# BarnitaSharma/Part-based-3D-Reconstruction

Measured on AMD Instinct MI355X. Metric: Mvoxel/s carved (semantic carve, 1024^3 grid), higher is better.
Workload: dtype u8

## Files before the change

### include/pb3d.h

```cpp
#ifndef PB3D_H
#define PB3D_H

#include <stddef.h>
#include <stdint.h>

#ifdef __cplusplus
extern "C" {
#endif

typedef struct pb3d_ctx pb3d_ctx;
typedef struct pb3d_event pb3d_event;

enum {
    PB3D_OK = 0,
    PB3D_EINVAL = -1,
    PB3D_ENODEVICE = -2,
    PB3D_ENOMEM = -3,
    PB3D_EUNSUPPORTED = -4,
    PB3D_ECOMM = -5,
    PB3D_EINDEX = -6
};

int pb3d_version(void);
const char* pb3d_last_error(void);
// ... 14 lines not shown
int pb3d_d2d(pb3d_ctx* ctx, void* dst, const void* src, size_t bytes);
int pb3d_event_create(pb3d_ctx* ctx, pb3d_event** ev);
int pb3d_event_record(pb3d_ctx* ctx, pb3d_event* ev);
int pb3d_event_elapsed_ms(pb3d_ctx* ctx, pb3d_event* start, pb3d_event* stop, float* ms);
void pb3d_event_destroy(pb3d_event* ev);

int pb3d_rotinv(int angle_deg, double M[9]);
int pb3d_offset(const double M[9], const int64_t shape[3], double off[3]);

int pb3d_carve_mask_dev(pb3d_ctx* ctx, const uint8_t* d_grid, int64_t W, int64_t H, int64_t D, int C,
                        const uint8_t* d_mask_wh, uint8_t* d_out);
int pb3d_carve_mask(pb3d_ctx* ctx, const uint8_t* grid, int64_t W, int64_t H, int64_t D, int C,
                    const uint8_t* mask_wh, uint8_t* out);

int pb3d_rotate_carve_dev(pb3d_ctx* ctx, const uint8_t* d_occ, int64_t W, int64_t H, int64_t D,
                          const double M[9], const double off[3], const uint8_t* d_mask_wh, uint8_t* d_out);
int pb3d_rotate_carve(pb3d_ctx* ctx, const uint8_t* occ, int64_t W, int64_t H, int64_t D,
                      const double M[9], const double off[3], const uint8_t* mask_wh, uint8_t* out);

int pb3d_process_grid_dev(pb3d_ctx* ctx, const uint8_t* d_occ, int64_t W, int64_t H, int64_t D,
                          const uint8_t* d_mask_wh, int angle_interval, uint8_t* d_out, uint8_t* d_tmp);
int pb3d_process_grid(pb3d_ctx* ctx, const uint8_t* occ, int64_t W, int64_t H, int64_t D,
                      const uint8_t* mask_wh, int angle_interval, uint8_t* out);

enum {
    PB3D_I8 = 1, PB3D_U8 = 2, PB3D_I16 = 3, PB3D_U16 = 4, PB3D_I32 = 5, PB3D_U32 = 6, PB3D_I64 = 7, PB3D_U64 = 8,
    PB3D_F32 = 9, PB3D_F64 = 10, PB3D_C64 = 11, PB3D_C128 = 12
};
size_t pb3d_dtype_bytes(int dtype);
int pb3d_process_grid_typed_dev(pb3d_ctx* ctx, const void* d_grid, int dtype, int64_t W, int64_t H, int64_t D, const uint8_t* d_mask_wh,
                                int angle_interval, void* d_out, void* d_tmp);

int pb3d_occupancy_dev(pb3d_ctx* ctx, const uint8_t* d_grid_rgb, int64_t nvox, uint8_t* d_occ);
int pb3d_occupancy(pb3d_ctx* ctx, const uint8_t* grid_rgb, int64_t nvox, uint8_t* occ);

int pb3d_color_apply_dev(pb3d_ctx* ctx, const uint8_t* d_carved, int64_t W, int64_t H, int64_t D,
                         const uint8_t* d_rgb_hw3, uint8_t* d_out);
int pb3d_color_apply(pb3d_ctx* ctx, const uint8_t* carved, int64_t W, int64_t H, int64_t D,
                     const uint8_t* rgb_hw3, uint8_t* out);

int pb3d_global_carve_dev(pb3d_ctx* ctx, const uint8_t* d_bin_hw, const uint8_t* d_rgb_hw3, int64_t h, int64_t w,
                          int angle_interval, int64_t x0, int64_t x1, uint8_t* d_out_slab);
int pb3d_global_carve(pb3d_ctx* ctx, const uint8_t* bin_hw, const uint8_t* rgb_hw3, int64_t h, int64_t w,
                      int angle_interval, uint8_t* out);

int pb3d_part_carve_dev(pb3d_ctx* ctx, const uint8_t* d_colored, int64_t W, int64_t H, int64_t D,
// ... 372 lines not shown
```

### part-based-3d-reconstruction_amd/csrc/ctx.hip

```cpp
#include <cmath>
#include <cstdlib>

#include <string>

#include "pb3d_internal.h"

static int pool_flush(pb3d_ctx* ctx);

static thread_local char g_err[512] = "";

void pb3d_set_error(const char* fmt, ...) {
    va_list ap;
    va_start(ap, fmt);
    vsnprintf(g_err, sizeof(g_err), fmt, ap);
    va_end(ap);
}

extern "C" {

int pb3d_version(void) { return 101; }

int64_t pb3d_sync_count(pb3d_ctx* ctx) { return ctx ? (int64_t)ctx->sync_count : -1; }

const char* pb3d_last_error(void) { return g_err; }
// ... 84 lines not shown
                (void)hipEventDestroy(ctx->s32_ev);
                (void)hipStreamDestroy(ctx->stream);
                free(ctx);
                return PB3D_EINVAL;
            }
        }
    }
    *out = ctx;
    return PB3D_OK;
}

namespace {
struct Knob { const char* name; int pb3d_ctx::*field; int lo, hi; const char* what; };
const Knob kKnobs[] = {
    {"sliced", &pb3d_ctx::tune_sliced, 0, 1, "0 (rotation steps on 0/1 data run bit-sliced) or 1 (never: byte chain)"},
    {"rot90_wide", &pb3d_ctx::tune_rot90_wide, 0, 2, "0 (choose), 1 or 2 (the 128-tile / 128-byte-segment kernels)"},
    {"rot90_fill", &pb3d_ctx::tune_rot90_fill, 0, 64, "a count of workgroups per CU (0 = the built-in rule)"},
    {"rot90_order", &pb3d_ctx::tune_rot90_order, 0, 1, "0 (a plane chunk per XCD) or 1 (plain x-fastest order)"},
    {"rot90_flat", &pb3d_ctx::tune_rot90_flat, 0, 2, "0 (choose), 1 (row-wise tile kernel) or 2 (flat on whole-line streams only)"},
    {"rot90_mask_block", &pb3d_ctx::tune_rot90_mask_block, 0, 1, "0 (mask bytes once into LDS) or 1 (per plane / segment)"},
    {"s32_gpw", &pb3d_ctx::tune_s32_gpw, 0, 1 << 20, "a count of plane groups"},
    {"s32_order", &pb3d_ctx::tune_s32_order, 0, 1, "0 (plane groups fastest) or 1 (x fastest)"},
    {"s32_fuse_last", &pb3d_ctx::tune_s32_fuse_last, 0, 1, "0 (fused) or 1 (table step)"},
    {"ccl_blocks", &pb3d_ctx::tune_ccl_blocks, 0, 1 << 20, "a count of workgroups per CU"},
    {"ccl_init_blocks", &pb3d_ctx::tune_ccl_init_blocks, 0, 1 << 20, "a count of workgroups per CU"},
    {"ccl_tilecols", &pb3d_ctx::tune_ccl_tilecols, 0, 64, "at most 64"},
    {"ccl_merge", &pb3d_ctx::tune_ccl_merge, 0, 1, "0 (tile kernels) or 1 (pairwise kernel)"},
    {"cluster_cell", &pb3d_ctx::tune_cluster_cell, 0, 2, "0 (the built-in rule), 1 (two points per cell) or 2 (cell edge above eps)"},
    {"cluster_timing", &pb3d_ctx::tune_cluster_timing, 0, 1, "0 or 1 (time the passes of a clustering with events)"},
    {"voxelize_timing", &pb3d_ctx::tune_voxelize_timing, 0, 1, "0 or 1 (time the two passes of a voxelization with events)"},
    {"render_timing", &pb3d_ctx::tune_render_timing, 0, 1, "0 or 1 (time the passes of a mesh rendering with events)"},
    {"iso_timing", &pb3d_ctx::tune_iso_timing, 0, 1, "0 or 1 (time the passes of an isosurface count and fill with events)"},
    {"simplify_timing", &pb3d_ctx::tune_simplify_timing, 0, 1, "0 or 1 (time the passes of a mesh simplification with events)"},
    {"inside_timing", &pb3d_ctx::tune_inside_timing, 0, 1, "0 or 1 (time the index build and the query of a containment test with events)"},
    {"inside_order", &pb3d_ctx::tune_inside_order, 0, 1, "0 (queries in input order) or 1 (in the cell order of the index)"},
    {"inside_table", &pb3d_ctx::tune_inside_table, 0, 1, "0 (set-ups recomputed from the corner table) or 1 (read from a table of finished set-ups)"},
    {"raycast_timing", &pb3d_ctx::tune_raycast_timing, 0, 1, "0 or 1 (time the index build and the query of a ray cast with events)"},
    {"raycast_stats", &pb3d_ctx::tune_raycast_stats, 0, 1, "0 or 1 (count hits, bad rays, face tests and cells of a ray cast for pb3d_cast_rays_last)"},
    {"orient_tile",&pb3d_ctx::tune_orient_tile, 0, 1, "0 (128-pixel tiles where they apply) or 1 (never)"},
    {"global_composed", &pb3d_ctx::tune_global_composed, 0, 1, "0 (mask bits -> sliced chain -> colours) or 1 (ones -> process -> colour)"},
    {"per_job", &pb3d_ctx::tune_per_job, 0, 1, "0 (merged / fused forms) or 1 (job by job)"},
    {"no_table_cache", &pb3d_ctx::tune_no_table_cache, 0, 1, "0 (tables cached across calls) or 1 (rebuilt every call)"},
    {"part90_inflight", &pb3d_ctx::tune_part90_inflight, 0, 44, "10 UA + UE with UA, UE in 1, 2, 4 (0 = the default 2 / 4)"},
    {"crop_ablate", &pb3d_ctx::tune_crop_ablate, 0, 1 << 20, "ablation switches of k_crop_chain"},
    {"uncap", &pb3d_ctx::tune_uncap, 0, 1, "0 or 1 (every grid-stride kernel as one workgroup per tile)"},
};
// ... 285 lines not shown
```

### part-based-3d-reconstruction_amd/csrc/pb3d_internal.h

```cpp
#pragma once
#include <hip/hip_runtime.h>

#include <cstdarg>
#include <cstdint>
#include <cstdio>
#include <cstring>
#include <initializer_list>
#include <type_traits>

#include "pb3d.h"

typedef uint8_t u8;
typedef int64_t i64;
typedef uint64_t u64;
typedef uint32_t u32;

enum pb3d_slot : int {
    PB3D_SLOT_HOST_IN0 = 0,
    PB3D_SLOT_HOST_OUT0 = 1,
    PB3D_SLOT_HOST_IN1 = 2,
    PB3D_SLOT_HOST_OUT1 = PB3D_SLOT_HOST_IN1,
    PB3D_SLOT_HOST_IN2 = 3,
    PB3D_SLOT_HOST_OUT2 = PB3D_SLOT_HOST_IN2,
    PB3D_SLOT_HOST_TMP = PB3D_SLOT_HOST_IN2,
// ... 241 lines not shown
    int device;
    int cus;
    hipStream_t stream;
    bool orient_lds_set;
    bool guided_lds_set;
    int tune_rot90_fill;
    int tune_rot90_order;
    int tune_rot90_flat;
    int tune_rot90_mask_block;
    int tune_orient_tile;
    int tune_global_composed;
    int tune_per_job;
    int tune_no_table_cache;
    int tune_part90_inflight;
    int tune_crop_ablate;
    int tune_uncap;
    int tune_sliced;
    int tune_rot90_wide;
    bool rot90w_lds_set;
    bool part90_lds_set;
    bool rot90wf_lds_set;
    int tune_s32_order;
    int tune_s32_fuse_last;
    int tune_s32_gpw;
    int tune_ccl_blocks;
    int tune_ccl_init_blocks;
    int tune_ccl_tilecols;
    int tune_ccl_merge;
    int tune_cluster_cell;
    int tune_cluster_timing;
    struct ClusterLast { bool valid, timed; float ms[5]; i64 cells[3]; } cluster_last;
    int tune_voxelize_timing;
    struct VoxelizeLast { bool valid, timed; float ms[2]; } voxelize_last;
    int tune_render_timing;
    struct RenderLast { bool valid, timed; float ms[5]; i64 stats[4]; } render_last;
    int tune_iso_timing;
    struct IsoLast { bool count_timed, fill_timed; float ms[4]; } iso_last;
    int tune_simplify_timing;
    struct SimplifyLast { bool valid, timed; float ms[5]; i64 counts[3]; } simplify_last;
    int tune_inside_timing;
    int tune_inside_order;
    int tune_inside_table;
    struct InsideLast { bool valid, timed; float ms[2]; i64 info[4]; } inside_last;
    int tune_raycast_timing;
    int tune_raycast_stats;
    struct RaycastLast { bool counted, timed; float ms[2]; i64 stats[6]; } raycast_last;
    void* scratch[PB3D_SLOT_COUNT];
    size_t scratch_bytes[PB3D_SLOT_COUNT];
    void* pinned;
    size_t pinned_bytes;
    void* stage;
    size_t stage_bytes, stage_head;
    u64 sync_count;
    struct PointsArgs { const void* grid; i64 A0, A1, A2, n, C, ncolors, stride; u8 colors[3 * 32]; };
    struct { pb3d_pair pair; PointsArgs a; } pts_dev, pts;
    struct MeshArgs { const void* grid; i64 A0, A1, A2, nv, nf, C, stride; };
    struct { pb3d_pair pair; MeshArgs a; } mesh_dev, mesh;
    struct IsoArgs { const void* vol; i64 n0, n1, n2, nv, nf; u64 level_bits, divisor_bits; };
    struct { pb3d_pair pair; IsoArgs a; } iso_dev, iso;
    struct { pb3d_pair pair; int ox, oy, oz; i64 X, Y, Z, n; } deform;
    struct ValidCache { void* buf; u64 gen; i64 W, D; double p[8]; } valid_cache;
    struct S32Cache { bool valid; u64 gen; i64 W, D; int ns; double p[32 * 8]; } s32_cache;
    hipEvent_t s32_ev;
    struct CclLast { bool valid; const void* labels; const void* bits; i64 rows, A2, P; u64 gen; bool members_only; int K, C; u32 colors[PB3D_CCL_MAX_COLORS]; } ccl_last;
    struct IcpIndex { bool valid; const void* tgt; i64 nt; int f64; u64 gen[3]; pb3d_nn_index ix; } icp_index;
    struct MeshGridLast { bool valid; i64 cells[3], entries, coarsenings; } mesh_grid_last;
    struct PoolBlock { void* p; size_t bytes; u64 stamp; };
    PoolBlock pool_free[PB3D_POOL_SLOTS];
    int pool_nfree;
    PoolBlock pool_live[PB3D_POOL_LIVE];
    int pool_nlive;
    size_t pool_cached, pool_cap;
    u64 pool_stamp;
    u64 scratch_gen;
    u64 scratch_slot_gen[PB3D_SLOT_COUNT];
    u64 scratch_use[PB3D_SLOT_COUNT];
    void* rccl_lib;
    void* rccl_comm;
    int rank, nranks;
};

void pb3d_set_error(const char* fmt, ...);

#define PB3D_HIP(call)                                                                          \
    do {                                                                                        \
// ... 159 lines not shown
```

### part-based-3d-reconstruction_amd/csrc/rot_common.h

```cpp
#pragma once
#include "pb3d_internal.h"

namespace {

struct RotParams {
    double m00, m01, m02, off0;
    double m20, m21, m22, off2;
};

struct Cell {
    double wx0, wx1, wz0, wz1;
    int s0, s2;
};

__device__ __forceinline__ double coord(double x, double z, double ma, double mb, double mc, double off) {
    double c = __dadd_rn(0.0, __dmul_rn(x, ma));
    c = __dadd_rn(c, __dmul_rn(0.0, mb));
    c = __dadd_rn(c, __dmul_rn(z, mc));
    return __dadd_rn(c, off);
}

__device__ __forceinline__ Cell make_cell(const RotParams& p, i64 x, i64 z, i64 W, i64 D) {
    Cell c;
    const double cc0 = coord((double)x, (double)z, p.m00, p.m01, p.m02, p.off0);
// ... 11 lines not shown
    return c;
}

__device__ __forceinline__ u32 lut_of(const Cell& c) {
    const double p00 = __dmul_rn(c.wx0, c.wz0), p01 = __dmul_rn(c.wx0, c.wz1), p10 = __dmul_rn(c.wx1, c.wz0),
                 p11 = __dmul_rn(c.wx1, c.wz1);
    u32 lut = 0;
#pragma unroll
    for (int b = 1; b < 16; ++b) {
        double acc = 0.0;
        if (b & 1) acc = __dadd_rn(acc, p00);
        if (b & 2) acc = __dadd_rn(acc, p01);
        if (b & 4) acc = __dadd_rn(acc, p10);
        if (b & 8) acc = __dadd_rn(acc, p11);
        if (acc > 0.0 && __dadd_rn(acc, 0.5) >= 1.0) lut |= 1u << b;
    }
    return lut;
}

__device__ __forceinline__ u32 bsel(u32 sel, u32 a, u32 b) { return (sel & a) | (~sel & b); }

__device__ __forceinline__ u32 sbit(u32 x, int k) { u32 r; asm("v_bfe_i32 %0, %1, %2, 1" : "=v"(r) : "v"(x), "n"(k)); return r; }
__device__ __forceinline__ u32 vbfi(u32 s, u32 a, u32 b) { u32 r; asm("v_bfi_b32 %0, %1, %2, %3" : "=v"(r) : "v"(s), "v"(a), "v"(b)); return r; }
__device__ __forceinline__ u32 lut_apply32(u32 lut, u32 t00, u32 t01, u32 t10, u32 t11) {
    u32 g[8], h[4];
    g[0] = vbfi(t00, sbit(lut, 1), sbit(lut, 0));   g[1] = vbfi(t00, sbit(lut, 3), sbit(lut, 2));
    g[2] = vbfi(t00, sbit(lut, 5), sbit(lut, 4));   g[3] = vbfi(t00, sbit(lut, 7), sbit(lut, 6));
    g[4] = vbfi(t00, sbit(lut, 9), sbit(lut, 8));   g[5] = vbfi(t00, sbit(lut, 11), sbit(lut, 10));
    g[6] = vbfi(t00, sbit(lut, 13), sbit(lut, 12)); g[7] = vbfi(t00, sbit(lut, 15), sbit(lut, 14));
#pragma unroll
    for (int j = 0; j < 4; ++j) h[j] = vbfi(t01, g[2 * j + 1], g[2 * j]);
    const u32 m0 = vbfi(t10, h[1], h[0]), m1 = vbfi(t10, h[3], h[2]);
    return vbfi(t11, m1, m0);
}

__device__ __forceinline__ u32 pperm(u32 hi, u32 lo, u32 sel) { return __builtin_amdgcn_perm(hi, lo, sel); }
__device__ __forceinline__ void tr4x4(u32 a0, u32 a1, u32 a2, u32 a3, u32 v[4]) {
    const u32 l01 = pperm(a1, a0, 0x05010400u), h01 = pperm(a1, a0, 0x07030602u);
    const u32 l23 = pperm(a3, a2, 0x05010400u), h23 = pperm(a3, a2, 0x07030602u);
    v[0] = pperm(l23, l01, 0x05040100u); v[1] = pperm(l23, l01, 0x07060302u);
    v[2] = pperm(h23, h01, 0x05040100u); v[3] = pperm(h23, h01, 0x07060302u);
}

}
```

### part-based-3d-reconstruction_amd/csrc/sliced.hip

```cpp
#include "rot_common.h"
#include "wave.h"

namespace {

typedef u32 u32x4 __attribute__((ext_vector_type(4)));
typedef u32 u32x2 __attribute__((ext_vector_type(2)));
typedef u32x2 u32x2_a1 __attribute__((aligned(1)));

constexpr int ST = 64;
constexpr int STHREADS = 256;
constexpr int SROWS = 96;
#ifndef PB3D_SPITCH
#define PB3D_SPITCH 101
#endif
constexpr int SPITCH = PB3D_SPITCH;
constexpr int SMAXU = 9;
constexpr int SMAXSTEPS = 32;

struct STile {
    int bx0, bz0, nrows, nunits, fits, pad0, pad1, pad2;
    u32 ugoff[SMAXU * STHREADS];
    unsigned short uloff[SMAXU * STHREADS];
    u32 cellw[16 * STHREADS];
};
static_assert(sizeof(STile) % 16 == 0, "STile is read with 16-byte loads");

struct StepParams { RotParams p[SMAXSTEPS]; };

__global__ __launch_bounds__(256) void k_s32_maskbits(const u8* __restrict__ mask_wh, i64 W, i64 H, int G, u32* __restrict__ bits, int* __restrict__ flag) {
    const i64 i = (i64)blockIdx.x * 256 + threadIdx.x;
    if (i == 0 && flag) *flag = 0;
    if (i >= (i64)G * W) return;
    const i64 g = i / W, x = i - g * W, y0 = 32 * g;
    u32 b = 0;
    if (y0 + 32 <= H) {
        typedef u32 u32x4_m1 __attribute__((ext_vector_type(4), aligned(1)));
        const u32x4_m1 lo = *(const u32x4_m1*)(mask_wh + x * H + y0), hi = *(const u32x4_m1*)(mask_wh + x * H + y0 + 16);
        const u32 w[8] = {lo.x, lo.y, lo.z, lo.w, hi.x, hi.y, hi.z, hi.w};
#pragma unroll
        for (int j = 0; j < 8; ++j) {
            const u32 t = w[j];
            const u32 z = (((t & 0x7f7f7f7fu) + 0x7f7f7f7fu) | t) & 0x80808080u;
            b |= (((z >> 7) * 0x01020408u) >> 24) << (4 * j);
// ... 285 lines not shown
            const u32 R = c[0], G = c[1], B = c[2];
            const u32 C0 = R | (G << 8) | (B << 16) | (R << 24), C1 = G | (B << 8) | (R << 16) | (G << 24), C2 = B | (R << 8) | (G << 16) | (B << 24);
#pragma unroll
            for (int j = 0; j < 4; ++j) rgb4((v[j][q >> 3] >> (q & 7)) & 0x01010101u, C0, C1, C2, o + 3 * j);
        }
        if (!fullrow) {
            if (live) {
                u8* dp = out + rowbase + (i64)q * D * 3 + 48 * zp;
                for (int bb = 0; bb < 48 && 3 * z + bb < 3 * D; ++bb) dp[bb] = (u8)(o[bb >> 2] >> (8 * (bb & 3)));
            }
            continue;
        }
#pragma unroll
        for (int k = 0; k < 3; ++k) { u32x4 t4; t4.x = o[4 * k]; t4.y = o[4 * k + 1]; t4.z = o[4 * k + 2]; t4.w = o[4 * k + 3]; win[wv][3 * lane + k] = t4; }
#pragma unroll
        for (int k = 0; k < 3; ++k) {
            const int cidx = 8 * k + zp;
            const u32x4 t4 = win[wv][grp + cidx];
            if (rowlive) *(u32x4_a1*)(out + rowbase + (i64)q * D * 3 + 16 * cidx) = t4;
        }
    }
}

__global__ __launch_bounds__(STHREADS) void k_s32_prep(StepParams sp, i64 W, i64 D, i64 Dp, int ntz, STile* __restrict__ tiles) {
    __shared__ int bb[4];
    __shared__ int rmin[SROWS], rmax[SROWS];
    __shared__ int ustart[SROWS + 1];
    __shared__ int rc0[SROWS];
    const int tid = threadIdx.x;
    const RotParams p = sp.p[blockIdx.y];
    const int t = (int)blockIdx.x;
    STile* o = tiles + (i64)blockIdx.y * gridDim.x + t;
    const i64 x0 = (i64)(t / ntz) * ST, z0 = (i64)(t % ntz) * ST;
    if (tid == 0) { bb[0] = 0x7fffffff; bb[1] = -1; bb[2] = 0x7fffffff; bb[3] = -1; }
    if (tid < SROWS) { rmin[tid] = 0x7fffffff; rmax[tid] = -1; }
    __syncthreads();
    const int tz = tid & 15, jr = tid >> 4;
    int s0[16], s2[16];
    u32 lut[16];
    int mn0 = 0x7fffffff, mx0 = -1, mn2 = 0x7fffffff, mx2 = -1;
#pragma unroll
    for (int i = 0; i < 4; ++i)
#pragma unroll
        for (int c = 0; c < 4; ++c) {
            const int k = 4 * i + c;
            const i64 x = x0 + jr + 16 * i, z = z0 + 4 * tz + c;
            s0[k] = -1; s2[k] = 0; lut[k] = 0;
            if (x < W && z < D) {
                const Cell cl = make_cell(p, x, z, W, D);
                if (cl.s0 >= 0) {
                    s0[k] = cl.s0; s2[k] = cl.s2;
                    lut[k] = lut_of(cl) | (cl.wx1 != 0.0 ? 1u << 16 : 0u) | (cl.wz1 != 0.0 ? 1u << 17 : 0u);
                    const int e0 = cl.s0 + (int)((lut[k] >> 16) & 1u), e2 = cl.s2 + (int)((lut[k] >> 17) & 1u);
                    mn0 = min(mn0, cl.s0); mx0 = max(mx0, e0); mn2 = min(mn2, cl.s2); mx2 = max(mx2, e2);
                }
            }
        }
// ... 24 lines not shown
                rc0[r] = 0;
                if (r < nrows && fits && rmax[r] >= 0) {
                    rc0[r] = (rmin[r] - bz0) >> 2;
                    n[h] = ((rmax[r] - bz0) >> 2) - ((rmin[r] - bz0) >> 2) + 1;
                }
            }
        }
        const int inc0 = wave_incl_scan(n[0]), inc1 = wave_incl_scan(n[1]);
        const int tot0 = __shfl(inc0, 63);
        ustart[tid] = inc0 - n[0];
        if (tid + 64 <= SROWS) ustart[tid + 64] = tot0 + inc1 - n[1];
    }
    __syncthreads();
    int nunits = (any_valid && fits) ? ustart[SROWS] : 0;
    if (nunits > SMAXU * STHREADS) { fits = false; nunits = 0; }
    if (fits && tid < nrows) {
        const int u0 = ustart[tid], u1 = ustart[tid + 1];
        for (int u = u0; u < u1; ++u) {
            const int cu = rc0[tid] + (u - u0);
            o->ugoff[u] = (u32)(((i64)bx0 + tid) * Dp + bz0 + 4 * cu);
            o->uloff[u] = (unsigned short)(tid * SPITCH + 4 * cu);
        }
    }
#pragma unroll
    for (int k = 0; k < 16; ++k) {
        u32 w = 0;
        if (fits && s0[k] >= 0) w = (lut[k] << 16) | (u32)((s0[k] - bx0) * SPITCH + (s2[k] - bz0));
        o->cellw[k * STHREADS + tid] = w;
    }
    if (tid == 0) { o->bx0 = bx0; o->bz0 = bz0; o->nrows = nrows; o->nunits = nunits; o->fits = fits ? 1 : 0; o->pad0 = o->pad1 = o->pad2 = 0; }
}

__global__ __launch_bounds__(STHREADS, 4) void k_s32_step(const u32* __restrict__ in, u32* __restrict__ out, const u32* __restrict__ mbits,
                                                           const STile* __restrict__ tiles, i64 W, i64 Dp, int G, int ntz, int ntiles, int gpw,
                                                           int nchunks) {
    __shared__ u32 tile[SROWS * SPITCH];
    const int tid = threadIdx.x;
    const int slot = (int)(blockIdx.x >> 3);
    const int t = slot % ntiles;
    const int chunk = (slot / ntiles) * 8 + (int)(blockIdx.x & 7u);
    if (chunk >= nchunks) return;
    const STile* ti = tiles + t;
    const i64 x0 = (i64)(t / ntz) * ST, z0 = (i64)(t % ntz) * ST;
    const int g_beg = chunk * gpw, g_end = g_beg + gpw < G ? g_beg + gpw : G;
    const int nunits = ti->nunits;
    u32 ug[SMAXU], ul[SMAXU];
#pragma unroll
    for (int j = 0; j < SMAXU; ++j) {
        const int u = tid + STHREADS * j;
        ug[j] = 0xffffffffu; ul[j] = 0;
        if (u < nunits) { ug[j] = ti->ugoff[u]; ul[j] = ti->uloff[u]; }
    }
    u32 cw[16];
#pragma unroll
    for (int i = 0; i < 16; ++i) cw[i] = ti->cellw[i * STHREADS + tid];
    const int tz = tid & 15, jr = tid >> 4;
    const i64 zc = z0 + 4 * tz;
    const bool zok = zc < Dp;
    u32x4 v[SMAXU];
    auto load_group = [&](int g) {
        const u32* src = in + (i64)g * W * Dp;
#pragma unroll
        for (int j = 0; j < SMAXU; ++j)
            if (ug[j] != 0xffffffffu) v[j] = *(const u32x4*)(src + ug[j]);
    };
    load_group(g_beg);
    for (int g = g_beg; g < g_end; ++g) {
#pragma unroll
        for (int j = 0; j < SMAXU; ++j)
            if (ug[j] != 0xffffffffu) { u32* d = tile + ul[j]; d[0] = v[j].x; d[1] = v[j].y; d[2] = v[j].z; d[3] = v[j].w; }
        __syncthreads();
        if (g + 1 < g_end) load_group(g + 1);
#pragma unroll
        for (int i = 0; i < 4; ++i) {
            u32 R[4];
#pragma unroll
            for (int c = 0; c < 4; ++c) {
                const u32 w = cw[4 * i + c];
                const u32* tp = tile + (w & 0xffffu);
                R[c] = lut_apply32(w >> 16, tp[0], tp[1], tp[SPITCH], tp[SPITCH + 1]);
            }
            const i64 x = x0 + jr + 16 * i;
            if (x < W && zok) {
                const u32 m = mbits[(i64)g * W + x];
                u32x4 r; r.x = R[0] & m; r.y = R[1] & m; r.z = R[2] & m; r.w = R[3] & m;
                *(u32x4*)(out + ((i64)g * W + x) * Dp + zc) = r;
            }
        }
        __syncthreads();
    }
}

static bool step_fits(const double M[9]) {
    const double ext0 = fabs(M[0]) + fabs(M[2]), ext2 = fabs(M[6]) + fabs(M[8]);
    return ext0 <= 1.4143 && ext2 <= 1.4143;
}

}

static int s32_chain(pb3d_ctx* ctx, const u8* d_occ, i64 W, i64 H, i64 D, const u8* d_mask_wh, int angle_interval, u8* d_out, const u8* d_rgb_hw3,
                     int known_binary, int* took, const double* Mx = nullptr, const double* offx = nullptr) {
    *took = 0;
    const int nrot = Mx ? 1 : 90 / angle_interval;
// ... 35 lines not shown
            const bool nt = W * H * D >= (i64)256 << 20;
#define PB3D_SLICE(WH, NTL) hipLaunchKernelGGL((k_s32_slice<WH, NTL>), dim3((total + 255u) / 256u), dim3(256), 0, ctx->stream, d_occ, (u32*)A, Mx ? (const u32*)nullptr : (const u32*)mb, W, H, D, Dp, mzb, mw, total, flag, mg, gfast)
            if (D % 16 == 0) { if (nt) PB3D_SLICE(true, true); else PB3D_SLICE(true, false); }
            else { if (nt) PB3D_SLICE(false, true); else PB3D_SLICE(false, false); }
#undef PB3D_SLICE
        } else {
            const u32 tq = (u32)((i64)G * W * (Dp / 4));
            hipLaunchKernelGGL(k_s32_fill, dim3((tq + 255u) / 256u), dim3(256), 0, ctx->stream, (u32*)A, (const u32*)mb, D, Dp, pb3d_make_magic((u32)(Dp / 4)), tq);
        }
        PB3D_CHECK_LAUNCH();
        int* hflag = (int*)((char*)ctx->pinned + pb3d_pinned_bytes - pb3d_pinned_flag);
        if (!known_binary) {
            PB3D_HIP(hipMemcpyAsync(hflag, flag, sizeof(int), hipMemcpyDeviceToHost, ctx->stream));
            PB3D_HIP(hipEventRecord(ctx->s32_ev, ctx->stream));
        }
        int gpw = ctx->tune_s32_gpw > 0 ? ctx->tune_s32_gpw : 1;
        if (ctx->tune_s32_gpw <= 0)
            while (gpw < G && (i64)ntiles * ((G + gpw - 1) / gpw) > (i64)ctx->cus * 16) ++gpw;
        const int nchunks = (G + gpw - 1) / gpw;
        const i64 nblk = 8ll * ntiles * ((nchunks + 7) / 8);
        PB3D_REQUIRE(nblk < (1ll << 31), "pb3d_process_grid: grid too large");
        u32 *src = (u32*)A, *dst = (u32*)B;
        bool checked = known_binary != 0;
        int nrot_tab = nrot;
        u32* vbits = nullptr;
        int vnw = 0, pc0 = 0, pc2 = 0;
        if (!Mx && nrot * angle_interval == 90 && ctx->tune_s32_fuse_last != 1 && H <= 65535ll * 32) {
            double M[9], off[3];
            PB3D_TRY(pb3d_rotinv(90, M));
            PB3D_TRY(pb3d_offset(M, shape, off));
            bool rot90 = false;
            if (pb3d_is_perm_step(M, off, W, D)) {
                PB3D_TRY(pb3d_perm_valid_table(ctx, M, off, W, D, &vbits, &vnw, &pc0, &pc2, &rot90));
                if (rot90) nrot_tab = nrot - 1; else vbits = nullptr;
            }
        }
        for (int s0 = 0; s0 < nrot_tab; s0 += SMAXSTEPS) {
            const int ns = nrot_tab - s0 < SMAXSTEPS ? nrot_tab - s0 : SMAXSTEPS;
            memset(&sp, 0, sizeof(sp));
            for (int k = 0; k < ns; ++k) {
                double M[9], off[3];
                if (Mx) { memcpy(M, Mx, sizeof(M)); memcpy(off, offx, sizeof(off)); }
                else {
                    PB3D_TRY(pb3d_rotinv((s0 + k + 1) * angle_interval, M));
                    PB3D_TRY(pb3d_offset(M, shape, off));
                }
                if (!step_fits(M)) return PB3D_EUNSUPPORTED;
                sp.p[k] = RotParams{M[0], M[1], M[2], off[0], M[6], M[7], M[8], off[2]};
            }
            void* tp;
            PB3D_TRY(pb3d_scratch(ctx, PB3D_SLOT_S32_TILE_PROGRAMS, (size_t)ns * ntiles * sizeof(STile), &tp));
            pb3d_ctx::S32Cache& sc = ctx->s32_cache;
            const bool hit = ctx->tune_no_table_cache != 1 && sc.valid && sc.gen == ctx->scratch_gen && sc.W == W && sc.D == D && sc.ns == ns &&
                             memcmp(sc.p, sp.p, sizeof(RotParams) * (size_t)ns) == 0;
            if (!hit) {
                sc.valid = false;
                hipLaunchKernelGGL(k_s32_prep, dim3((unsigned)ntiles, (unsigned)ns), dim3(STHREADS), 0, ctx->stream, sp, W, D, Dp, ntz, (STile*)tp);
                PB3D_CHECK_LAUNCH();
                static_assert(sizeof(sc.p) == sizeof(sp.p), "S32Cache holds one StepParams");
                memcpy(sc.p, sp.p, sizeof(sp.p));
                sc.W = W; sc.D = D; sc.ns = ns; sc.gen = ctx->scratch_gen; sc.valid = nrot_tab <= SMAXSTEPS;
            }
            for (int k = 0; k < ns; ++k) {
                hipLaunchKernelGGL(k_s32_step, dim3((unsigned)nblk), dim3(STHREADS), 0, ctx->stream, (const u32*)src, dst, (const u32*)mb,
                                   (const STile*)tp + (i64)k * ntiles, W, Dp, G, ntz, ntiles, gpw, nchunks);
                u32* t2 = src; src = dst; dst = t2;
            }
            PB3D_CHECK_LAUNCH();
        }
        if (vbits && d_rgb_hw3) {
            const int utz = (int)((D + UZ - 1) / UZ), utx = (int)((W + UX - 1) / UX);
            hipLaunchKernelGGL(k_s32_unslice90_rgb, dim3((unsigned)(utz * utx), (unsigned)G), dim3(256), 0, ctx->stream, (const u32*)src, d_out, d_rgb_hw3,
                               (const u32*)mb, (const u32*)vbits, vnw, W, H, D, Dp, pc0, pc2, utz);
        } else if (vbits) {
            const int utz = (int)((D + UZ - 1) / UZ), utx = (int)((W + UX - 1) / UX);
            hipLaunchKernelGGL(k_s32_unslice90, dim3((unsigned)(utz * utx), (unsigned)G), dim3(256), 0, ctx->stream, (const u32*)src, d_out, (const u32*)mb,
                               (const u32*)vbits, vnw, W, H, D, Dp, pc0, pc2, utz);
        } else if (d_rgb_hw3)
            hipLaunchKernelGGL(k_s32_unslice_rgb, dim3((total + 255u) / 256u), dim3(256), 0, ctx->stream, (const u32*)src, d_out, d_rgb_hw3, W, H, D, Dp, mzb, mw,
                               total);
        else
// ... 8 lines not shown
    };
    rc = body();
    (void)pb3d_dev_free(ctx, A);
    (void)pb3d_dev_free(ctx, B);
    if (rc == PB3D_EUNSUPPORTED) return PB3D_OK;
    if (rc == PB3D_OK) *took = 1;
    return rc;
}

int pb3d_process_grid_sliced(pb3d_ctx* ctx, const u8* d_occ, i64 W, i64 H, i64 D, const u8* d_mask_wh, int angle_interval, u8* d_out,
                             int known_binary, int* took) {
    return s32_chain(ctx, d_occ, W, H, D, d_mask_wh, angle_interval, d_out, nullptr, known_binary, took);
}

int pb3d_global_carve_sliced(pb3d_ctx* ctx, const u8* d_mask_wh, const u8* d_rgb_hw3, i64 W, i64 H, i64 D, int angle_interval, u8* d_out_rgb,
                             int* took) {
    return s32_chain(ctx, nullptr, W, H, D, d_mask_wh, angle_interval, d_out_rgb, d_rgb_hw3, 1, took);
}

int pb3d_rotate_step_sliced(pb3d_ctx* ctx, const u8* d_occ, i64 W, i64 H, i64 D, const double M[9], const double off[3], const u8* d_mask_wh, u8* d_out,
                            int* took) {
    return s32_chain(ctx, d_occ, W, H, D, d_mask_wh, 90, d_out, nullptr, 0, took, M, off);
}
```

### part-based-3d-reconstruction_amd/pb3d/_lib.py

```python
import ctypes as C
import os
import threading

import numpy as np

_HERE = os.path.dirname(os.path.abspath(__file__))
LIB_PATH = os.environ.get("PB3D_LIB_PATH") or os.path.join(_HERE, "libpb3d.so")

u8p = C.POINTER(C.c_uint8)
i64 = C.c_int64
i64p = C.POINTER(C.c_int64)
dblp = C.POINTER(C.c_double)
intp = C.POINTER(C.c_int)
vp = C.c_void_p

_SIGNATURES = {
    "pb3d_version": [],
    "pb3d_last_error": [],
    "pb3d_device_count": [intp],
    "pb3d_create": [C.c_int, C.POINTER(vp)],
    "pb3d_destroy": [vp],
    "pb3d_make_current": [vp],
    "pb3d_device_info": [vp, C.c_char_p, C.c_int, intp, i64p],
    "pb3d_sync": [vp],
    "pb3d_set_tuning": [vp, C.c_char_p, C.c_int],
    "pb3d_dev_alloc": [vp, C.c_size_t, C.POINTER(vp)],
    "pb3d_dev_free": [vp, vp],
    "pb3d_dev_memset": [vp, vp, C.c_int, C.c_size_t],
    "pb3d_h2d": [vp, vp, vp, C.c_size_t],
    "pb3d_d2h": [vp, vp, vp, C.c_size_t],
    "pb3d_h2d_async": [vp, vp, vp, C.c_size_t],
    "pb3d_sync_count": [vp],
    "pb3d_d2d": [vp, vp, vp, C.c_size_t],
    "pb3d_event_create": [vp, C.POINTER(vp)],
    "pb3d_event_record": [vp, vp],
    "pb3d_event_elapsed_ms": [vp, vp, vp, C.POINTER(C.c_float)],
    "pb3d_event_destroy": [vp],
    "pb3d_rotinv": [C.c_int, dblp],
    "pb3d_offset": [dblp, i64p, dblp],
    "pb3d_carve_mask_dev": [vp, vp, i64, i64, i64, C.c_int, vp, vp],
    "pb3d_carve_mask": [vp, u8p, i64, i64, i64, C.c_int, u8p, u8p],
    "pb3d_rotate_carve_dev": [vp, vp, i64, i64, i64, dblp, dblp, vp, vp],
    "pb3d_rotate_carve": [vp, u8p, i64, i64, i64, dblp, dblp, u8p, u8p],
    "pb3d_process_grid_dev": [vp, vp, i64, i64, i64, vp, C.c_int, vp, vp],
    "pb3d_process_grid": [vp, u8p, i64, i64, i64, u8p, C.c_int, u8p],
    "pb3d_dtype_bytes": [C.c_int],
    "pb3d_process_grid_typed_dev": [vp, vp, C.c_int, i64, i64, i64, vp, C.c_int, vp, vp],
    "pb3d_occupancy_dev": [vp, vp, i64, vp],
    "pb3d_occupancy": [vp, u8p, i64, u8p],
    "pb3d_color_apply_dev": [vp, vp, i64, i64, i64, vp, vp],
    "pb3d_color_apply": [vp, u8p, i64, i64, i64, u8p, u8p],
    "pb3d_global_carve_dev": [vp, vp, vp, i64, i64, C.c_int, i64, i64, vp],
    "pb3d_global_carve": [vp, u8p, u8p, i64, i64, C.c_int, u8p],
    "pb3d_part_carve_dev": [vp, vp, i64, i64, i64, vp, vp, intp, intp, C.c_int, vp],
    "pb3d_part_carve": [vp, u8p, i64, i64, i64, u8p, u8p, intp, intp, C.c_int, u8p],
    "pb3d_points_count_dev": [vp, vp, i64, i64, i64, C.c_int, u8p, C.c_int, C.c_int, i64p],
    "pb3d_points_fill_dev": [vp, vp, i64, i64, i64, C.c_int, u8p, C.c_int, C.c_int, i64, vp, vp],
    "pb3d_points_extract_dev": [vp, vp, i64, i64, i64, C.c_int, u8p, C.c_int, i64, vp, vp, i64p],
    "pb3d_points_count": [vp, u8p, i64, i64, i64, C.c_int, u8p, C.c_int, C.c_int, i64p],
    "pb3d_points_fill": [vp, i64, C.POINTER(C.c_float), u8p],
    "pb3d_mesh_count_dev": [vp, vp, i64, i64, i64, C.c_int, C.c_int, i64p, i64p],
    "pb3d_mesh_fill_dev": [vp, vp, i64, i64, i64, C.c_int, C.c_int, i64, i64, vp, vp, vp, vp],
    "pb3d_mesh_colors_dev": [vp, vp, i64, i64, i64, C.c_int, C.c_int, vp, i64, vp],
    "pb3d_mesh_count": [vp, u8p, i64, i64, i64, C.c_int, C.c_int, i64p, i64p],
    "pb3d_mesh_fill": [vp, i64, i64, vp, vp, vp, vp],
    "pb3d_iso_count_resident": [vp, vp, i64, i64, i64, C.c_double, C.c_float, i64p, i64p],
    "pb3d_iso_fill_resident": [vp, vp, i64, i64, i64, C.c_double, C.c_float, i64, i64, vp, vp],
    "pb3d_iso_count": [vp, vp, i64, i64, i64, C.c_double, C.c_float, i64p, i64p],
# ... 131 lines not shown
    "pb3d_render_last_ms": [vp, dblp],
    "pb3d_cast_rays_resident": [vp, vp, vp, C.c_int, i64, vp, C.c_int, i64, vp, C.c_int, i64, C.c_double, C.c_double, C.c_int, vp, vp, vp, vp],
    "pb3d_cast_rays_last": [vp, i64p],
    "pb3d_cast_rays_last_ms": [vp, dblp],
}
class IouRow(C.Structure):
    _fields_ = [("pred", vp), ("gt", vp), ("gate", vp), ("pred_bits", C.c_uint32), ("gt_bits", C.c_uint32), ("gate_bits", C.c_uint32)]


_VIEW_FIELDS = [("R", C.c_double * 9), ("cam", C.c_double * 3), ("f", C.c_double), ("cx", C.c_double), ("cy", C.c_double),
                ("prec", C.c_int * 4), ("Himg", C.c_int), ("Wimg", C.c_int)]


class CarveView(C.Structure):
    _fields_ = _VIEW_FIELDS + [("d_maskbits", vp)]


class PaintView(C.Structure):
    _fields_ = _VIEW_FIELDS + [("d_image", vp), ("d_zbuf", vp)]


PRESENCE_BYTES = 1 << 21

_RESTYPES = {"pb3d_dtype_bytes": C.c_size_t, "pb3d_sync_count": C.c_int64, "pb3d_last_error": C.c_char_p, "pb3d_destroy": None, "pb3d_event_destroy": None}

EXPORTED_SYMBOLS = tuple(_SIGNATURES)

_lib = None
_ctx = None
_lock = threading.Lock()


class Pb3dError(RuntimeError):
    pass


def load():
    global _lib
    if _lib is None:
        if not os.path.exists(LIB_PATH):
            raise ImportError(f"{LIB_PATH} is missing: build it with `python -c 'import __graft_entry__ as g; g.build()'` "
                              "(pb3d has no CPU fallback)")
        lib = C.CDLL(LIB_PATH)
        for name, args in _SIGNATURES.items():
            fn = getattr(lib, name)
            fn.argtypes = args
            fn.restype = _RESTYPES.get(name, C.c_int)
# ... 18 lines not shown


def default_device():
    for key in ("PB3D_DEVICE", "LOCAL_RANK"):
        if os.environ.get(key, "").isdigit():
            return int(os.environ[key])
    return 0


def ctx():
    global _ctx
    with _lock:
        if _ctx is None:
            h = vp()
            check(load().pb3d_create(default_device(), C.byref(h)))
            _ctx = h
    return _ctx


def set_tuning(name, value):
    check(load().pb3d_set_tuning(ctx(), name.encode(), int(value)))


def reset():
    global _ctx
    with _lock:
        if _ctx is not None:
            load().pb3d_destroy(_ctx)
            _ctx = None


def _ptr(b):
    if b is None or isinstance(b, C.c_void_p):
        return b
    return C.c_void_p(b.ptr)


def p_u8(a):
    return a.ctypes.data_as(u8p)


def p_dbl(a):
    return a.ctypes.data_as(dblp)


def as_u8(a, what):
# ... 9 lines not shown
```

Baseline: 1.142 million.

## Use canonical tile programs in bit-sliced rotation step for common 4-input tables

Classifies each cell's 16-bit lookup table in the prep kernel as one of eight canonical forms (selecting a corner or majority/threshold functions), and when all cells of a wave qualify, the step kernel evaluates them with a short bitop3/bfi sequence instead of the general 15-instruction mux tree. Cell words now store byte offsets plus a 3-bit code, with a zeroed LDS pad for empty cells. It also adds counters and API calls reporting canonical versus general waves. This adds wave-uniform branching and prep work, and only helps when the interpolation tables match the canonical set.

```diff
diff --git a/include/pb3d.h b/include/pb3d.h
--- a/include/pb3d.h
+++ b/include/pb3d.h
@@ -60,6 +60,9 @@
                           const uint8_t* d_mask_wh, int angle_interval, uint8_t* d_out, uint8_t* d_tmp);
 int pb3d_process_grid(pb3d_ctx* ctx, const uint8_t* occ, int64_t W, int64_t H, int64_t D,
                       const uint8_t* mask_wh, int angle_interval, uint8_t* out);
+int pb3d_s32_last_build(pb3d_ctx* ctx, int64_t* n_canonical_waves, int64_t* n_general_waves);
+int pb3d_s32_canon_of(uint32_t table16, uint32_t* code);
+uint32_t pb3d_s32_canon_table(uint32_t code);
 
 enum {
     PB3D_I8 = 1, PB3D_U8 = 2, PB3D_I16 = 3, PB3D_U16 = 4, PB3D_I32 = 5, PB3D_U32 = 6, PB3D_I64 = 7, PB3D_U64 = 8,
diff --git a/part-based-3d-reconstruction_amd/csrc/ctx.hip b/part-based-3d-reconstruction_amd/csrc/ctx.hip
--- a/part-based-3d-reconstruction_amd/csrc/ctx.hip
+++ b/part-based-3d-reconstruction_amd/csrc/ctx.hip
@@ -130,6 +130,7 @@
     {"s32_gpw", &pb3d_ctx::tune_s32_gpw, 0, 1 << 20, "a count of plane groups"},
     {"s32_order", &pb3d_ctx::tune_s32_order, 0, 1, "0 (plane groups fastest) or 1 (x fastest)"},
     {"s32_fuse_last", &pb3d_ctx::tune_s32_fuse_last, 0, 1, "0 (fused) or 1 (table step)"},
+    {"s32_tree", &pb3d_ctx::tune_s32_tree, 0, 1, "0 (canonical tile programs where the tables allow) or 1 (the general tree everywhere)"},
     {"ccl_blocks", &pb3d_ctx::tune_ccl_blocks, 0, 1 << 20, "a count of workgroups per CU"},
     {"ccl_init_blocks", &pb3d_ctx::tune_ccl_init_blocks, 0, 1 << 20, "a count of workgroups per CU"},
     {"ccl_tilecols", &pb3d_ctx::tune_ccl_tilecols, 0, 64, "at most 64"},
diff --git a/part-based-3d-reconstruction_amd/csrc/pb3d_internal.h b/part-based-3d-reconstruction_amd/csrc/pb3d_internal.h
--- a/part-based-3d-reconstruction_amd/csrc/pb3d_internal.h
+++ b/part-based-3d-reconstruction_amd/csrc/pb3d_internal.h
@@ -287,6 +287,7 @@
     bool rot90wf_lds_set;
     int tune_s32_order;
     int tune_s32_fuse_last;
+    int tune_s32_tree;
     int tune_s32_gpw;
     int tune_ccl_blocks;
     int tune_ccl_init_blocks;
@@ -325,7 +326,8 @@
     struct { pb3d_pair pair; IsoArgs a; } iso_dev, iso;
     struct { pb3d_pair pair; int ox, oy, oz; i64 X, Y, Z, n; } deform;
     struct ValidCache { void* buf; u64 gen; i64 W, D; double p[8]; } valid_cache;
-    struct S32Cache { bool valid; u64 gen; i64 W, D; int ns; double p[32 * 8]; } s32_cache;
+    struct S32Cache { bool valid; u64 gen; i64 W, D; int ns, tree; double p[32 * 8]; } s32_cache;
+    bool s32_built;
     hipEvent_t s32_ev;
     struct CclLast { bool valid; const void* labels; const void* bits; i64 rows, A2, P; u64 gen; bool members_only; int K, C; u32 colors[PB3D_CCL_MAX_COLORS]; } ccl_last;
     struct IcpIndex { bool valid; const void* tgt; i64 nt; int f64; u64 gen[3]; pb3d_nn_index ix; } icp_index;
diff --git a/part-based-3d-reconstruction_amd/csrc/rot_common.h b/part-based-3d-reconstruction_amd/csrc/rot_common.h
--- a/part-based-3d-reconstruction_amd/csrc/rot_common.h
+++ b/part-based-3d-reconstruction_amd/csrc/rot_common.h
@@ -57,16 +57,41 @@
 
 __device__ __forceinline__ u32 sbit(u32 x, int k) { u32 r; asm("v_bfe_i32 %0, %1, %2, 1" : "=v"(r) : "v"(x), "n"(k)); return r; }
 __device__ __forceinline__ u32 vbfi(u32 s, u32 a, u32 b) { u32 r; asm("v_bfi_b32 %0, %1, %2, %3" : "=v"(r) : "v"(s), "v"(a), "v"(b)); return r; }
+template <int B = 0>
 __device__ __forceinline__ u32 lut_apply32(u32 lut, u32 t00, u32 t01, u32 t10, u32 t11) {
     u32 g[8], h[4];
-    g[0] = vbfi(t00, sbit(lut, 1), sbit(lut, 0));   g[1] = vbfi(t00, sbit(lut, 3), sbit(lut, 2));
-    g[2] = vbfi(t00, sbit(lut, 5), sbit(lut, 4));   g[3] = vbfi(t00, sbit(lut, 7), sbit(lut, 6));
-    g[4] = vbfi(t00, sbit(lut, 9), sbit(lut, 8));   g[5] = vbfi(t00, sbit(lut, 11), sbit(lut, 10));
-    g[6] = vbfi(t00, sbit(lut, 13), sbit(lut, 12)); g[7] = vbfi(t00, sbit(lut, 15), sbit(lut, 14));
+    g[0] = vbfi(t00, sbit(lut, B + 1), sbit(lut, B + 0));   g[1] = vbfi(t00, sbit(lut, B + 3), sbit(lut, B + 2));
+    g[2] = vbfi(t00, sbit(lut, B + 5), sbit(lut, B + 4));   g[3] = vbfi(t00, sbit(lut, B + 7), sbit(lut, B + 6));
+    g[4] = vbfi(t00, sbit(lut, B + 9), sbit(lut, B + 8));   g[5] = vbfi(t00, sbit(lut, B + 11), sbit(lut, B + 10));
+    g[6] = vbfi(t00, sbit(lut, B + 13), sbit(lut, B + 12)); g[7] = vbfi(t00, sbit(lut, B + 15), sbit(lut, B + 14));
 #pragma unroll
     for (int j = 0; j < 4; ++j) h[j] = vbfi(t01, g[2 * j + 1], g[2 * j]);
     const u32 m0 = vbfi(t10, h[1], h[0]), m1 = vbfi(t10, h[3], h[2]);
     return vbfi(t11, m1, m0);
+}
+
+__host__ __device__ inline u32 canon_table(u32 code) {
+    switch (code & 7u) {
+        case 0: return 0xeaa8u; case 1: return 0xecc8u; case 2: return 0xf8e0u; case 3: return 0xfe80u;
+        case 4: return 0xaaaau; case 5: return 0xccccu; case 6: return 0xf0f0u; default: return 0xff00u;
+    }
+}
+__host__ __device__ inline bool canon_of(u32 table16, u32* code) {
+    switch (table16) {
+        case 0xeaa8u: *code = 0; return true; case 0xecc8u: *code = 1; return true; case 0xf8e0u: *code = 2; return true; case 0xfe80u: *code = 3; return true;
+        case 0xaaaau: *code = 4; return true; case 0xccccu: *code = 5; return true; case 0xf0f0u: *code = 6; return true; case 0xff00u: *code = 7; return true;
+        default: return false;
+    }
+}
+template <int TT>
+__device__ __forceinline__ u32 bitop3(u32 a, u32 b, u32 c) { return __builtin_amdgcn_bitop3_b32(a, b, c, TT); }
+template <int B>
+__device__ __forceinline__ u32 canon_apply32(u32 w, u32 t00, u32 t01, u32 t10, u32 t11) {
+    const u32 sz = sbit(w, B), sx = sbit(w, B + 1), K = sbit(w, B + 2);
+    const u32 a = vbfi(sx, vbfi(sz, t11, t10), vbfi(sz, t01, t00));
+    const u32 m = bitop3<0xe8>(t00, t01, t10), p = bitop3<0x96>(t00, t01, t10);
+    const u32 ge2 = bitop3<0xf8>(m, p, t11), ge3 = bitop3<0xe0>(m, p, t11);
+    return vbfi(K, a, vbfi(a, ge2, ge3));
 }
 
 __device__ __forceinline__ u32 pperm(u32 hi, u32 lo, u32 sel) { return __builtin_amdgcn_perm(hi, lo, sel); }
diff --git a/part-based-3d-reconstruction_amd/csrc/sliced.hip b/part-based-3d-reconstruction_amd/csrc/sliced.hip
--- a/part-based-3d-reconstruction_amd/csrc/sliced.hip
+++ b/part-based-3d-reconstruction_amd/csrc/sliced.hip
@@ -16,9 +16,14 @@
 constexpr int SPITCH = PB3D_SPITCH;
 constexpr int SMAXU = 9;
 constexpr int SMAXSTEPS = 32;
+constexpr int SZERO = SROWS * SPITCH;
+constexpr int SLDS = (SZERO + SPITCH + 2 + 3) & ~3;
+static_assert(4 * SLDS * 4 <= 160 * 1024, "four workgroups of k_s32_step share a CU's LDS");
+static_assert(4 * (SZERO + SPITCH + 1) < 65536, "canonical cell words hold a 16-bit byte offset");
+constexpr int SCODE = 16;
 
 struct STile {
-    int bx0, bz0, nrows, nunits, fits, pad0, pad1, pad2;
+    int bx0, bz0, nrows, nunits, fits, canon, pad1, pad2;
     u32 ugoff[SMAXU * STHREADS];
     unsigned short uloff[SMAXU * STHREADS];
     u32 cellw[16 * STHREADS];
@@ -350,8 +355,10 @@
     }
 }
 
-__global__ __launch_bounds__(STHREADS) void k_s32_prep(StepParams sp, i64 W, i64 D, i64 Dp, int ntz, STile* __restrict__ tiles) {
+__global__ __launch_bounds__(STHREADS) void k_s32_prep(StepParams sp, i64 W, i64 D, i64 Dp, int ntz, STile* __restrict__ tiles, int tree,
+                                                       u32* __restrict__ nwaves) {
     __shared__ int bb[4];
+    __shared__ int cmask;
     __shared__ int rmin[SROWS], rmax[SROWS];
     __shared__ int ustart[SROWS + 1];
     __shared__ int rc0[SROWS];
@@ -360,7 +367,7 @@
     const int t = (int)blockIdx.x;
     STile* o = tiles + (i64)blockIdx.y * gridDim.x + t;
     const i64 x0 = (i64)(t / ntz) * ST, z0 = (i64)(t % ntz) * ST;
-    if (tid == 0) { bb[0] = 0x7fffffff; bb[1] = -1; bb[2] = 0x7fffffff; bb[3] = -1; }
+    if (tid == 0) { bb[0] = 0x7fffffff; bb[1] = -1; bb[2] = 0x7fffffff; bb[3] = -1; cmask = 0; }
     if (tid < SROWS) { rmin[tid] = 0x7fffffff; rmax[tid] = -1; }
     __syncthreads();
     const int tz = tid & 15, jr = tid >> 4;
@@ -431,19 +438,38 @@
             o->uloff[u] = (unsigned short)(tid * SPITCH + 4 * cu);
         }
     }
+    bool mine = tree == 0 && fits, live = false;
 #pragma unroll
     for (int k = 0; k < 16; ++k) {
-        u32 w = 0;
-        if (fits && s0[k] >= 0) w = (lut[k] << 16) | (u32)((s0[k] - bx0) * SPITCH + (s2[k] - bz0));
+        u32 code;
+        if (s0[k] >= 0) live = true;
+        if (s0[k] >= 0 && !canon_of(lut[k] & 0xffffu, &code)) mine = false;
+    }
+    const bool canon = __all(mine) != 0;
+    const bool counts = __any(live && fits) != 0;
+    if ((tid & 63) == 0) {
+        if (canon) atomicOr(&cmask, 1 << (tid >> 6));
+        if (nwaves && counts) atomicAdd(nwaves + (canon ? 0 : 1), 1u);
+    }
+#pragma unroll
+    for (int k = 0; k < 16; ++k) {
+        u32 w = canon ? (u32)(4 * SZERO) | (4u << SCODE) : 0u;
+        if (fits && s0[k] >= 0) {
+            const u32 off = (u32)((s0[k] - bx0) * SPITCH + (s2[k] - bz0));
+            u32 code = 0;
+            (void)canon_of(lut[k] & 0xffffu, &code);
+            w = ((canon ? code : lut[k]) << SCODE) | (4u * off);
+        }
         o->cellw[k * STHREADS + tid] = w;
     }
-    if (tid == 0) { o->bx0 = bx0; o->bz0 = bz0; o->nrows = nrows; o->nunits = nunits; o->fits = fits ? 1 : 0; o->pad0 = o->pad1 = o->pad2 = 0; }
+    __syncthreads();
+    if (tid == 0) { o->bx0 = bx0; o->bz0 = bz0; o->nrows = nrows; o->nunits = nunits; o->fits = fits ? 1 : 0; o->canon = cmask; o->pad1 = o->pad2 = 0; }
 }
 
 __global__ __launch_bounds__(STHREADS, 4) void k_s32_step(const u32* __restrict__ in, u32* __restrict__ out, const u32* __restrict__ mbits,
                                                            const STile* __restrict__ tiles, i64 W, i64 Dp, int G, int ntz, int ntiles, int gpw,
                                                            int nchunks) {
-    __shared__ u32 tile[SROWS * SPITCH];
+    __shared__ u32 tile[SLDS];
     const int tid = threadIdx.x;
     const int slot = (int)(blockIdx.x >> 3);
     const int t = slot % ntiles;
@@ -453,6 +479,8 @@
     const i64 x0 = (i64)(t / ntz) * ST, z0 = (i64)(t % ntz) * ST;
     const int g_beg = chunk * gpw, g_end = g_beg + gpw < G ? g_beg + gpw : G;
     const int nunits = ti->nunits;
+    const bool canon = ((__builtin_amdgcn_readfirstlane(ti->canon) >> __builtin_amdgcn_readfirstlane(tid >> 6)) & 1) != 0;
+    if (tid < SLDS - SZERO) tile[SZERO + tid] = 0u;
     u32 ug[SMAXU], ul[SMAXU];
 #pragma unroll
     for (int j = 0; j < SMAXU; ++j) {
@@ -481,13 +509,24 @@
         __syncthreads();
         if (g + 1 < g_end) load_group(g + 1);
 #pragma unroll
+        for (int i = 0; i < 16; ++i) asm volatile("" : "+v"(cw[i]));
+#pragma unroll
         for (int i = 0; i < 4; ++i) {
             u32 R[4];
-#pragma unroll
-            for (int c = 0; c < 4; ++c) {
-                const u32 w = cw[4 * i + c];
-                const u32* tp = tile + (w & 0xffffu);
-                R[c] = lut_apply32(w >> 16, tp[0], tp[1], tp[SPITCH], tp[SPITCH + 1]);
+            if (canon) {
+#pragma unroll
+                for (int c = 0; c < 4; ++c) {
+                    const u32 w = cw[4 * i + c];
+                    const u32* tp = (const u32*)((const char*)tile + (w & 0xffffu));
+                    R[c] = canon_apply32<SCODE>(w, tp[0], tp[1], tp[SPITCH], tp[SPITCH + 1]);
+                }
+            } else {
+#pragma unroll
+                for (int c = 0; c < 4; ++c) {
+                    const u32 w = cw[4 * i + c];
+                    const u32* tp = (const u32*)((const char*)tile + (w & 0xffffu));
+                    R[c] = lut_apply32<SCODE>(w, tp[0], tp[1], tp[SPITCH], tp[SPITCH + 1]);
+                }
             }
             const i64 x = x0 + jr + 16 * i;
             if (x < W && zok) {
@@ -569,6 +608,9 @@
         PB3D_REQUIRE(nblk < (1ll << 31), "pb3d_process_grid: grid too large");
         u32 *src = (u32*)A, *dst = (u32*)B;
         bool checked = known_binary != 0;
+        const int tree = ctx->tune_s32_tree == 1 ? 1 : 0;
+        u32* nwaves = (u32*)flag + 4;
+        bool counted = false;
         int nrot_tab = nrot;
         u32* vbits = nullptr;
         int vnw = 0, pc0 = 0, pc2 = 0;
@@ -599,11 +641,15 @@
             PB3D_TRY(pb3d_scratch(ctx, PB3D_SLOT_S32_TILE_PROGRAMS, (size_t)ns * ntiles * sizeof(STile), &tp));
             pb3d_ctx::S32Cache& sc = ctx->s32_cache;
             const bool hit = ctx->tune_no_table_cache != 1 && sc.valid && sc.gen == ctx->scratch_gen && sc.W == W && sc.D == D && sc.ns == ns &&
-                             memcmp(sc.p, sp.p, sizeof(RotParams) * (size_t)ns) == 0;
+                             sc.tree == tree && memcmp(sc.p, sp.p, sizeof(RotParams) * (size_t)ns) == 0;
             if (!hit) {
                 sc.valid = false;
-                hipLaunchKernelGGL(k_s32_prep, dim3((unsigned)ntiles, (unsigned)ns), dim3(STHREADS), 0, ctx->stream, sp, W, D, Dp, ntz, (STile*)tp);
+                if (!counted) { PB3D_HIP(hipMemsetAsync(nwaves, 0, 2 * sizeof(u32), ctx->stream)); counted = true; }
+                hipLaunchKernelGGL(k_s32_prep, dim3((unsigned)ntiles, (unsigned)ns), dim3(STHREADS), 0, ctx->stream, sp, W, D, Dp, ntz, (STile*)tp, tree,
+                                   nwaves);
                 PB3D_CHECK_LAUNCH();
+                ctx->s32_built = true;
+                sc.tree = tree;
                 static_assert(sizeof(sc.p) == sizeof(sp.p), "S32Cache holds one StepParams");
                 memcpy(sc.p, sp.p, sizeof(sp.p));
                 sc.W = W; sc.D = D; sc.ns = ns; sc.gen = ctx->scratch_gen; sc.valid = nrot_tab <= SMAXSTEPS;
@@ -658,3 +704,20 @@
                             int* took) {
     return s32_chain(ctx, d_occ, W, H, D, d_mask_wh, 90, d_out, nullptr, 0, took, M, off);
 }
+
+int pb3d_s32_last_build(pb3d_ctx* ctx, int64_t* n_canonical_waves, int64_t* n_general_waves) {
+    PB3D_REQUIRE(ctx != nullptr && n_canonical_waves != nullptr && n_general_waves != nullptr, "pb3d_s32_last_build: null argument");
+    PB3D_REQUIRE(ctx->s32_built && ctx->scratch[PB3D_SLOT_SLICED_FLAG] != nullptr, "pb3d_s32_last_build: no tile programs have been built on this context");
+    u32 n[2];
+    PB3D_TRY(pb3d_read_back(ctx, n, (const u32*)ctx->scratch[PB3D_SLOT_SLICED_FLAG] + 4, sizeof(n)));
+    *n_canonical_waves = n[0]; *n_general_waves = n[1];
+    return PB3D_OK;
+}
+
+int pb3d_s32_canon_of(uint32_t table16, uint32_t* code) {
+    u32 c = 0;
+    const bool ok = canon_of(table16, &c);
+    if (ok && code) *code = c;
+    return ok ? 1 : 0;
+}
+uint32_t pb3d_s32_canon_table(uint32_t code) { return canon_table(code & 7u); }
diff --git a/part-based-3d-reconstruction_amd/pb3d/_lib.py b/part-based-3d-reconstruction_amd/pb3d/_lib.py
--- a/part-based-3d-reconstruction_amd/pb3d/_lib.py
+++ b/part-based-3d-reconstruction_amd/pb3d/_lib.py
@@ -44,6 +44,9 @@
     "pb3d_rotate_carve": [vp, u8p, i64, i64, i64, dblp, dblp, u8p, u8p],
     "pb3d_process_grid_dev": [vp, vp, i64, i64, i64, vp, C.c_int, vp, vp],
     "pb3d_process_grid": [vp, u8p, i64, i64, i64, u8p, C.c_int, u8p],
+    "pb3d_s32_last_build": [vp, i64p, i64p],
+    "pb3d_s32_canon_of": [C.c_uint32, C.POINTER(C.c_uint32)],
+    "pb3d_s32_canon_table": [C.c_uint32],
     "pb3d_dtype_bytes": [C.c_int],
     "pb3d_process_grid_typed_dev": [vp, vp, C.c_int, i64, i64, i64, vp, C.c_int, vp, vp],
     "pb3d_occupancy_dev": [vp, vp, i64, vp],
@@ -221,7 +224,7 @@
 
 PRESENCE_BYTES = 1 << 21
 
-_RESTYPES = {"pb3d_dtype_bytes": C.c_size_t, "pb3d_sync_count": C.c_int64, "pb3d_last_error": C.c_char_p, "pb3d_destroy": None, "pb3d_event_destroy": None}
+_RESTYPES = {"pb3d_dtype_bytes": C.c_size_t, "pb3d_s32_canon_table": C.c_uint32, "pb3d_sync_count": C.c_int64, "pb3d_last_error": C.c_char_p, "pb3d_destroy": None, "pb3d_event_destroy": None}
 
 EXPORTED_SYMBOLS = tuple(_SIGNATURES)
 
@@ -286,6 +289,12 @@
     check(load().pb3d_set_tuning(ctx(), name.encode(), int(value)))
 
 
+def s32_last_build():
+    nc, ng = C.c_int64(0), C.c_int64(0)
+    check(load().pb3d_s32_last_build(ctx(), C.byref(nc), C.byref(ng)))
+    return nc.value, ng.value
+
+
 def reset():
     global _ctx
     with _lock:
```

Measured after the change: 1.154 million (median of 6 runs). No clear change (+1.0%).
